# atoms-ufrj/atomsmm

Measured on AMD Instinct MI355X. Metric: ns/day on 100k-atom TIP3P RESPA box; near-nonbonded HBM GB/s vs 8 TB/s peak, higher is better.
Workload: dtype f64

## Files before the change

### atomsmm_amd/csrc/cluster.hip

```cpp
#include <algorithm>
#include <cmath>
#include <cstdio>
#include <cstdlib>
#include <cstring>
#include <type_traits>
#include <vector>

#include "amm_ctx.h"
#include "bonded_terms.h"
#include "cluster.h"
#include "device_utils.h"
#include "pair_math.h"
#include "pair_tab.h"

#ifndef AMM_EXP_NOLJ
#define AMM_EXP_NOLJ 0
#endif

__device__ double amm_erfcx_table_dev_c[AMM_ERFCX_NI * AMM_ERFCX_NC];
static bool g_erfcx_uploaded_c[64] = {false};

void amm_cluster_classify(int n, const std::vector<int> &ptr, const std::vector<int> &idx, std::vector<int> &mol_first, std::vector<int> &rest) {
    mol_first.clear();
    rest.clear();
// ... 813 lines not shown
                    const int T = __builtin_amdgcn_readfirstlane(s_cnt[0][t] + s_cnt[1][t] + s_cnt[2][t] + s_cnt[3][t]);
                    const int nch = (T + 127) >> 7;
                    const int have = __builtin_amdgcn_readlane(row_cnt, t);
                    int nf = have & 0xffff, nb_ = (int)((unsigned)have >> 16);
                    int *row_out = nl + (size_t)(tb + t - c_begin) * cap;
                    for (int k = 0; k < nch; ++k) {
                        const int j = j0 + k;
                        const int cc = __builtin_amdgcn_readfirstlane(s_ccnt[j]);
                        const int cn = cc & 0xffff, cf = (int)((unsigned)cc >> 16);
                        if ((j & 3) == w && nf + nb_ + cn + cf <= cap) {
                            for (int i = lane; i < cn; i += 64) row_out[nf + i] = s_stage[j][i];
                            for (int i = lane; i < cf; i += 64) row_out[cap - 1 - nb_ - i] = s_stage[j][127 - i];
                        }
                        nf = min(nf + cn, 0xffff);
                        nb_ = min(nb_ + cf, 0xffff);
                    }
                    row_cnt = lane == t ? (nf | (nb_ << 16)) : row_cnt;
                    j0 += nch;
                }
                CBS_STAMP(5);
                __syncthreads();
                CBS_STAMP(6);
            }
            if (w == 0 && lane < nt) {
                const int count = row_cnt & 0xffff, countf = (int)((unsigned)row_cnt >> 16);
                const int total_nb = count + countf;
                const bool over = total_nb > cap;
                nnb[tb + lane - c_begin] = over ? 0 : total_nb;
                nnb_near[tb + lane - c_begin] = over ? 0 : count;
                if (over) flags[1] = 1;
                wsum += (unsigned long long)total_nb;
                wnear += (unsigned long long)count;
                wmax = max(wmax, total_nb);
            }
        }
    }
    __syncthreads();
    }
    for (int off = 32; off > 0; off >>= 1) {
        wsum += __shfl_xor(wsum, off);
        wnear += __shfl_xor(wnear, off);
        wmax = max(wmax, __shfl_xor(wmax, off));
    }
    if (w == 0 && lane == 0) {
        amm_st_l2(&blockstats[3 * blockIdx.x], wsum);
        amm_st_l2(&blockstats[3 * blockIdx.x + 1], (unsigned long long)wmax);
        amm_st_l2(&blockstats[3 * blockIdx.x + 2], wnear);
    }
    if (amm_last_block(ticket)) cfinish_build_block(flags, counters, blockstats, (int)gridDim.x, 0);
}

#define AMM_CPHASES 6
struct CPairArgs {
    int c_begin, nrows, lpa_shift, cap;
    const int *aperm;
    const int *nl, *nnb, *nnb_total;
    const double4 *posq;
    const double2 *lj;
    double *force;
    int accumulate, sorted_out;
    Box box;
    const double *host_tab;
    int host_bytes;
    double margin;
    int ntask;
    int per_pair_image;
    int rpx, nphase;
    int ph_off[AMM_CPHASES], ph_shift[AMM_CPHASES], ph_ntask[AMM_CPHASES];
#ifdef AMM_CPAIR_TIMING
    unsigned long long *wave_times;
#endif
    const double *host_tab_ss;
    int host_ss_bytes, host_ss_off, site_atoms;
    double hsig_site, seps2_site;
    const double *guest_tab, *guest_tab_ss;
    int guest_bytes, guest_ss_bytes, guest_ss_off, g_accumulate;
    const double *tab_image;
    unsigned long long host_serial, guest_serial;
    PairForce *tab_owner;
    double *gforce;
    double gfac, gsr;
};

#ifdef AMM_CPAIR_TIMING
#define CWALK_T_PARAM , unsigned long long &t_first
#define CWALK_T_ARG , t_first
#else
#define CWALK_T_PARAM
#define CWALK_T_ARG
#endif
template <int FAM, int CMODE, int GFAM, int IMG, int SMASK>
__device__ __forceinline__ void cwalk_rows(const CPairArgs &A, const PairConsts &c, const PairConsts &g, const char *tabh, const char *tabg,
                                           const double *erfcx, const double4 (&pi)[3], const double2 *li, int i_sites, const int (&so)[3],
                                           const int (&sog)[3], double sign_lj, const int *row, int nfront, int nn, int sub, int lpa,
                                           int self, double (&f)[9], double (&fg)[9] CWALK_T_PARAM) {
    constexpr bool DUAL = GFAM >= 0;
    constexpr bool SS = SMASK != 0;
    const int back = A.cap - 1 + nfront;
    const double r2low = DUAL ? fmax(c.tab.r2min, g.tab.r2min) : c.tab.r2min;
    const double r2low_ss = DUAL ? fmax(c.tab.ss_r2min, g.tab.ss_r2min) : c.tab.ss_r2min;
    auto entry = [&](int k) { return k < nn ? row[k < nfront ? k : back - k] : self; };
    auto load_pos = [&](int e, int b) {
        return *reinterpret_cast<const double4 *>(reinterpret_cast<const char *>(A.posq) + (size_t)((unsigned)e & 0x1fffffffu) * 96u + 32 * b);
    };
    auto load_lj = [&](int e, int b) {
        double2 l = make_double2(0.0, 0.0);
        if (i_sites != 0 && __builtin_amdgcn_ballot_w64((((unsigned)e >> 29) >> b) & 1u) != 0ull)
            l = *reinterpret_cast<const double2 *>(reinterpret_cast<const char *>(A.lj) + (size_t)((unsigned)e & 0x1fffffffu) * 48u + 16 * b);
        return l;
    };
    double4 pj[3];
    double2 lj[3];
    int k = sub;
    int e = entry(k), en = entry(k + lpa);
#pragma unroll
    for (int b = 0; b < 3; ++b) {
        pj[b] = load_pos(e, b);
        if (!SS) lj[b] = load_lj(e, b);
    }
    while (__builtin_amdgcn_ballot_w64(k < nn) != 0ull) {
        const bool ok = k < nn;
        const bool front = k < nfront;
        const bool any_front = DUAL && __builtin_amdgcn_ballot_w64(front) != 0ull;
        const unsigned bits = (unsigned)e >> 29;
        const int e2 = entry(k + 2 * lpa);
        double sx = 0.0, sy = 0.0, sz = 0.0;
        if (IMG == 1) {
            sx = A.box.L[0] * rint((pj[0].x - pi[0].x) * A.box.invL[0]);
            sy = A.box.L[1] * rint((pj[0].y - pi[0].y) * A.box.invL[1]);
            sz = A.box.L[2] * rint((pj[0].z - pi[0].z) * A.box.invL[2]);
        }
#pragma unroll
        for (int b = 0; b < 3; ++b) {
            const double xb = pj[b].x - sx, yb = pj[b].y - sy, zb = pj[b].z - sz, qb = pj[b].w;
            const int mb = SS ? -(int)((bits >> b) & 1u) : 0;
            double dx[3], dy[3], dz[3], r2[3], fr[3], gl[3];
            {
                TabLookup th[3];
#pragma unroll
                for (int a = 0; a < 3; ++a) {
                    dx[a] = pi[a].x - xb;
                    dy[a] = pi[a].y - yb;
                    dz[a] = pi[a].z - zb;
                    if (IMG == 2) {
                        dx[a] = amm_min_image(dx[a], A.box.L[0], A.box.invL[0]);
                        dy[a] = amm_min_image(dy[a], A.box.L[1], A.box.invL[1]);
                        dz[a] = amm_min_image(dz[a], A.box.L[2], A.box.invL[2]);
                    }
                    r2[a] = dx[a] * dx[a] + dy[a] * dy[a] + dz[a] * dz[a];
                    th[a] = amm_tab_fetch(tabh, c.tab, r2[a], ((SMASK >> a) & 1) ? (unsigned)(so[a] & mb) : 0u);
                    if (DUAL) gl[a] = 0.0;
                }
                __builtin_amdgcn_sched_barrier(0);
#pragma unroll
                for (int a = 0; a < 3; ++a) fr[a] = (pi[a].w * qb) * amm_tab_horner(th[a]);
            }
            if (!SS && !AMM_EXP_NOLJ && i_sites != 0 && __builtin_amdgcn_ballot_w64(ok && ((bits >> b) & 1u)) != 0ull) {
#pragma unroll
                for (int a = 0; a < 3; ++a)
                    if ((i_sites >> a) & 1) {
                        const double2 la = li[64 * a];
                        const double sig = la.x + lj[b].x, eps4 = la.y * lj[b].y;
                        const LJCommon L = amm_lj_common(r2[a], sig, eps4);
                        fr[a] = amm_sum_unfused(fr[a], amm_lj_force<FAM, CMODE>(c, L, sig, eps4));
                        if (DUAL && any_front) {
                            LJCommon Lg = L;
                            Lg.dlj_r *= A.gsr;
                            gl[a] = amm_lj_force<(DUAL ? GFAM : FAM), 0>(g, Lg, sig, eps4 * A.gsr);
                        }
                    }
            }
            bool any_low = false;
            bool lowp[3];
#pragma unroll
            for (int a = 0; a < 3; ++a) {
                bool low = r2[a] < r2low;
                if ((SMASK >> a) & 1) low = low || ((so[a] & mb) != 0 && r2[a] < r2low_ss);
                lowp[a] = low;
                const bool pass = ok && (r2[a] < c.rc2);
                any_low = any_low || (ok && low);
                const double fh = (pass && !low) ? fr[a] : 0.0;
                f[3 * a] += fh * dx[a];
                f[3 * a + 1] += fh * dy[a];
                f[3 * a + 2] += fh * dz[a];
            }
            if (DUAL) {
                __builtin_amdgcn_sched_barrier(0);
                if (any_front) {
                    TabLookup tg[3];
#pragma unroll
                    for (int a = 0; a < 3; ++a) tg[a] = amm_tab_fetch(tabg, g.tab, r2[a], ((SMASK >> a) & 1) ? (unsigned)(sog[a] & mb) : 0u);
                    __builtin_amdgcn_sched_barrier(0);
#pragma unroll
                    for (int a = 0; a < 3; ++a) {
                        const double gr = amm_sum_unfused(((pi[a].w * qb) * A.gfac) * amm_tab_horner(tg[a]), gl[a]);
                        const bool pass = front && (r2[a] < g.rc2) && !lowp[a];
                        const double gh = pass ? gr : 0.0;
                        fg[3 * a] += gh * dx[a];
                        fg[3 * a + 1] += gh * dy[a];
                        fg[3 * a + 2] += gh * dz[a];
                    }
                }
            }
            if (__builtin_amdgcn_ballot_w64(any_low) != 0ull) {
                for (int a = 0; a < 3; ++a) {
                    const bool low = ok && lowp[a];
                    double sg, e4;
                    if (SS) {
                        const bool both = ((SMASK >> a) & 1) && (so[a] & mb) != 0;
                        sg = 2.0 * A.hsig_site;
                        e4 = both ? A.seps2_site * A.seps2_site * sign_lj : 0.0;
                    } else {
                        const double2 lx = A.lj[3 * ((unsigned)e & 0x1fffffffu) + b];
                        const double2 la = li[64 * a];
                        sg = la.x + lx.x;
                        e4 = la.y * lx.y;
                    }
                    double e_, fr_;
                    amm_pair_math<FAM, CMODE, false, false>(c, low ? r2[a] : 1.0, pi[a].w * qb, sg, e4, e_, fr_, erfcx);
                    fr_ = (low && r2[a] < c.rc2) ? fr_ : 0.0;
                    f[3 * a] += fr_ * dx[a];
                    f[3 * a + 1] += fr_ * dy[a];
                    f[3 * a + 2] += fr_ * dz[a];
                    if (DUAL) {
                        double gr_;
                        amm_pair_math<(DUAL ? GFAM : FAM), 0, false, false>(g, low ? r2[a] : 1.0, (pi[a].w * qb) * A.gfac, sg, e4 * A.gsr, e_, gr_, erfcx);
                        gr_ = (low && front && r2[a] < g.rc2) ? gr_ : 0.0;
                        fg[3 * a] += gr_ * dx[a];
                        fg[3 * a + 1] += gr_ * dy[a];
                        fg[3 * a + 2] += gr_ * dz[a];
                    }
                }
            }
            pj[b] = load_pos(en, b);
            if (!SS) lj[b] = load_lj(en, b);
        }
        e = en;
        en = e2;
        k += lpa;
#ifdef AMM_CPAIR_TIMING
        if (!t_first) t_first = wall_clock64();
#endif
    }
}

struct CEpiPre {
    const double *a, *b;
    double coef;
    int plus;
};
struct CEpiArgs {
    int niter, npre;
    int recompute_f0;
    double *x, *v, *f0;
    const double *mass;
    double c1, d, c2;
    CEpiPre pre[AMM_MAX_PRE];
    const int *cperm;
    const int4 *term_l;
    const double4 *term_q;
    const unsigned long long *atom_recs;
    int *spec_count, *spec_clear, *spec_members, *spec_start, *spec_flags, *spec_ticket;
    int spec_capc;
    CellGrid grid;
    double *xchg_x, *xchg_v;
    int c_first;
    double4 *posq_next;
    double2 *lj_next;
    const double *q_next, *hsig_next, *seps2_next;
    WatchArgs W;
};

#ifndef CEPI_INLINE
#define CEPI_INLINE __forceinline__
#endif

struct CEpiArgs;
template <int Q>
__device__ __forceinline__ double cquad_bcast(double v) {
    constexpr int ctrl = Q | (Q << 2) | (Q << 4) | (Q << 6);
    const long long b = __double_as_longlong(v);
    const int lo = __builtin_amdgcn_mov_dpp((int)(b & 0xffffffffll), ctrl, 0xf, 0xf, true);
    const int hi = __builtin_amdgcn_mov_dpp((int)(b >> 32), ctrl, 0xf, 0xf, true);
    return __longlong_as_double(((long long)hi << 32) | (unsigned int)lo);
}

struct PosTermRegs {
// ... 182 lines not shown
            AMM_CEPI_TERM(2)
            AMM_CEPI_TERM(3)
#undef AMM_CEPI_TERM
        }
        if (it >= 0) {
#pragma clang fp contract(off)
#pragma unroll
            for (int j = 0; j < 3; ++j) {
                const double num = E.c2 * f[j];
                const double dv = amm_div_mass(num, m, rm, rok);
                v[j] = v[j] + dv;
            }
        }
    }
    CEPI_STAMP(2);
    if (has) {
#pragma unroll
        for (int j = 0; j < 3; ++j) {
            if (E.niter == 0) E.x[3 * a + j] = x[j];
            E.v[3 * a + j] = v[j];
            E.f0[3 * a + j] = f[j];
        }
        if (E.xchg_x) {
            const size_t sl = 3 * (size_t)(cs - E.c_first) + l;
#pragma unroll
            for (int j = 0; j < 3; ++j) {
                if (E.niter == 0) E.xchg_x[3 * sl + j] = x[j];
                E.xchg_v[3 * sl + j] = v[j];
            }
        }
    }
}

template <int BS>
__device__ __forceinline__ int cscan_counts(int ncell, const int *count, int *start) {
    __shared__ int s_part[BS / 64], s_most[BS / 64];
    const int t = threadIdx.x, lane = t & 63, w = t >> 6;
    const int per = (ncell + BS - 1) / BS;
    const int c0 = min(t * per, ncell), c1 = min(c0 + per, ncell);
    int sum = 0, most = 0;
    for (int c = c0; c < c1; ++c) {
        const int v = amm_ld_l2(&count[c]);
        sum += v;
        most = max(most, v);
    }
    int incl = sum;
    for (int off = 1; off < 64; off <<= 1) {
        const int up = __shfl_up(incl, off);
        if (lane >= off) incl += up;
        most = max(most, __shfl_xor(most, off));
    }
    if (lane == 63) {
        s_part[w] = incl;
        s_most[w] = most;
    }
    __syncthreads();
    int base = 0, all_most = 0;
#pragma unroll
    for (int k = 0; k < BS / 64; ++k) {
        if (k < w) base += s_part[k];
        all_most = max(all_most, s_most[k]);
    }
    int run = base + incl - sum;
    for (int c = c0; c < c1; ++c) {
        start[c] = run;
        run += amm_ld_l2(&count[c]);
    }
    if (t == BS - 1) start[ncell] = run;
    return all_most;
}

#ifndef AMM_CBS_SINGLE
#define AMM_CBS_SINGLE 512
#endif

#ifndef AMM_CBS_NEAR
#define AMM_CBS_NEAR 512
#endif
#ifndef AMM_CTAB_WAVES_PER_EU
#define AMM_CTAB_WAVES_PER_EU 1
#endif
template <int FAM, int CMODE, int GFAM, int BS, int SMASK, bool EPI = false>
__global__ void __launch_bounds__(BS) __attribute__((amdgpu_waves_per_eu(AMM_CTAB_WAVES_PER_EU)))
k_cpair(CPairArgs A, PairConsts c, PairConsts g, CEpiArgs E) {
    constexpr bool DUAL = GFAM >= 0;
    constexpr bool SS = SMASK != 0;
    extern __shared__ __align__(16) char s_lds[];
    if (EPI && E.spec_clear) {
        for (int cidx = blockIdx.x * BS + threadIdx.x; cidx <= E.grid.ncell; cidx += gridDim.x * BS) E.spec_clear[cidx] = 0;
    }
#ifdef AMM_CPAIR_TIMING
    const unsigned long long t_entry = wall_clock64();
    unsigned long long t_staged = 0, t_first = 0;
    int n_tasks_done = 0, n_interior = 0;
    unsigned long long t_epi[3] = {0, 0, 0};
#endif
    constexpr int WPB = BS / 64;
    const int lane = threadIdx.x & 63;
    const double sign = c.sign;
    const int xcd = blockIdx.x & 7, nwx = (gridDim.x >> 3) * WPB;
    const int row_end = min((xcd + 1) * A.rpx, A.nrows);
#ifdef AMM_CPAIR_SWAP
    const int wave = (int)(threadIdx.x >> 6) ^ 4;
#else
    const int wave = (int)(threadIdx.x >> 6);
#endif
    const int task0 = (int)(blockIdx.x >> 3) * WPB + __builtin_amdgcn_readfirstlane(wave);
    int phase = 0, task = task0;
    auto seek = [&]() {
        while (phase < A.nphase && task >= A.ph_ntask[phase]) {
            ++phase;
            task = task0;
        }
        return phase < A.nphase;
    };
    constexpr bool AHEAD = SS;
    int shift = 0, lpa = 1, sub = 0, a = 0, cs = 0, nfront = 0, nn = 0;
    bool valid = false;
    const int *row = nullptr;
    double4 pi[3];
    double2 pl[3];
    auto pre_rows = [&]() {
        shift = A.ph_shift[phase];
        lpa = 1 << shift;
        sub = lane & (lpa - 1);
        a = xcd * A.rpx + A.ph_off[phase] + task * (64 >> shift) + (lane >> shift);
        valid = a < row_end;
        cs = A.c_begin + (valid ? a : 0);
#pragma unroll
        for (int t = 0; t < 3; ++t) {
            pi[t] = A.posq[3 * cs + t];
            pl[t] = A.lj[3 * cs + t];
        }
        nfront = valid ? A.nnb[a] : 0;
        nn = valid ? (A.nnb_total ? A.nnb_total[a] : nfront) : 0;
        row = A.nl + (size_t)(valid ? a : 0) * A.cap;
    };
    bool has = seek();
    if (AHEAD && has) pre_rows();

    const int used = A.host_bytes + (DUAL ? A.guest_bytes : 0) + (SS ? A.host_ss_bytes + (DUAL ? A.guest_ss_bytes : 0) : 0);
    double2 tabs[(160 * 1024) / (BS * 16)];
    amm_stage_issue<BS>(tabs, A.tab_image, used);
    amm_stage_commit<BS>(tabs, s_lds, used);
    amm_stage_rest<BS>(tabs, A.tab_image, s_lds, used);
#if defined(AMM_EXP_TAB_GLOBAL)
    const char *tabh = reinterpret_cast<const char *>(A.host_tab);
#else
    const char *tabh = s_lds;
#endif
    const char *tabg = s_lds + A.host_bytes;
    const double *erfcx = amm_erfcx_table_dev_c;
    double2 *s_li = nullptr;
    if (!SS) {
        double *s_erfcx = reinterpret_cast<double *>(s_lds + used);
        for (int k = threadIdx.x; k < AMM_ERFCX_NI * AMM_ERFCX_NC; k += BS) s_erfcx[k] = amm_erfcx_table_dev_c[k];
        erfcx = s_erfcx;
        s_li = reinterpret_cast<double2 *>(s_erfcx + AMM_ERFCX_NI * AMM_ERFCX_NC) + (threadIdx.x >> 6) * 192;
    }
    __syncthreads();
#ifdef AMM_CPAIR_TIMING
    t_staged = wall_clock64();
#endif

    PairConsts c1 = c, g1 = g;
    c1.sign = 1.0;
    g1.sign = 1.0;
    while (has) {
        if (!AHEAD) pre_rows();
        const int t_a = a, t_cs = cs, t_sub = sub, t_lpa = lpa;
        const bool t_valid = valid;
        int i_sites = 0;
        int so[3] = {0, 0, 0}, sog[3] = {0, 0, 0};
        if (!SS) __builtin_amdgcn_wave_barrier();
#pragma unroll
        for (int t = 0; t < 3; ++t) {
            pi[t].w *= c.Kc * sign;
            double2 l = pl[t];
            l.y *= sign;
            if (!SS) s_li[64 * t + lane] = l;
            const bool site = valid && l.y != 0.0;
            if ((SMASK >> t) & 1) {
                so[t] = site ? A.host_ss_off : 0;
                if (DUAL) sog[t] = site ? A.guest_ss_off : 0;
            }
            if (__builtin_amdgcn_ballot_w64(site) != 0ull) i_sites |= 1 << t;
        }
        if (!SS) {
            __builtin_amdgcn_fence(__ATOMIC_RELEASE, "wavefront");
            __builtin_amdgcn_wave_barrier();
            __builtin_amdgcn_fence(__ATOMIC_ACQUIRE, "wavefront");
        }
        const double2 *li = SS ? nullptr : s_li + lane;
        const bool edge = valid && !(pi[0].x >= A.margin && pi[0].x <= A.box.L[0] - A.margin && pi[0].y >= A.margin &&
                                     pi[0].y <= A.box.L[1] - A.margin && pi[0].z >= A.margin && pi[0].z <= A.box.L[2] - A.margin);
        const bool interior = __builtin_amdgcn_ballot_w64(edge) == 0ull;
#ifdef AMM_CPAIR_TIMING
        ++n_tasks_done;
        n_interior += interior ? 1 : 0;
#endif
        double f[9], fg[9];
#pragma unroll
        for (int k = 0; k < 9; ++k) f[k] = fg[k] = 0.0;
        if (A.per_pair_image) cwalk_rows<FAM, CMODE, GFAM, 2, SMASK>(A, c1, g1, tabh, tabg, erfcx, pi, li, i_sites, so, sog, sign, row, nfront, nn, sub, lpa, cs, f, fg CWALK_T_ARG);
        else if (interior) cwalk_rows<FAM, CMODE, GFAM, 0, SMASK>(A, c1, g1, tabh, tabg, erfcx, pi, li, i_sites, so, sog, sign, row, nfront, nn, sub, lpa, cs, f, fg CWALK_T_ARG);
        else cwalk_rows<FAM, CMODE, GFAM, 1, SMASK>(A, c1, g1, tabh, tabg, erfcx, pi, li, i_sites, so, sog, sign, row, nfront, nn, sub, lpa, cs, f, fg CWALK_T_ARG);
        task += nwx;
        has = seek();
        if (AHEAD && has) pre_rows();
        for (int off = t_lpa >> 1; off > 0; off >>= 1) {
#pragma unroll
            for (int k = 0; k < 9; ++k) {
                f[k] += __shfl_xor(f[k], off);
                if (DUAL) fg[k] += __shfl_xor(fg[k], off);
            }
        }
        if (t_valid && t_sub == 0) {
#pragma unroll
            for (int t = 0; t < 3; ++t) {
                const int i = A.sorted_out ? 3 * t_a + t : A.aperm[3 * t_cs + t];
#pragma unroll
                for (int d = 0; d < 3; ++d) {
                    if (A.accumulate) A.force[3 * i + d] += f[3 * t + d];
                    else A.force[3 * i + d] = f[3 * t + d];
                    if (DUAL) {
                        if (A.g_accumulate) A.gforce[3 * i + d] += fg[3 * t + d];
                        else A.gforce[3 * i + d] = fg[3 * t + d];
                    }
                }
            }
        }
    }
#ifdef AMM_CPAIR_TIMING
    if (EPI) t_staged = wall_clock64();
#endif
    if (EPI) {
        for (int phase = 0; phase < A.nphase; ++phase) {
            const int shift = A.ph_shift[phase], row0 = xcd * A.rpx + A.ph_off[phase], ntask = A.ph_ntask[phase];
            const int rpw = 64 >> shift;
            for (int task = (int)(blockIdx.x >> 3) * WPB + (int)(threadIdx.x >> 6); task < ntask; task += nwx) {
                const int a = row0 + task * rpw + (lane >> shift);
                const bool valid = a < row_end;
#ifdef AMM_CPAIR_TIMING
                cepi_rows(E, A.box, A.c_begin + (valid ? a : 0), valid, lane & ((1 << shift) - 1), t_epi);
#else
                cepi_rows(E, A.box, A.c_begin + (valid ? a : 0), valid, lane & ((1 << shift) - 1));
#endif
            }
        }
        if (E.spec_count && amm_last_block(E.spec_ticket)) {
            if (amm_ld_l2(&E.spec_flags[0])) {
                const int fullest = cscan_counts<BS>(E.grid.ncell, E.spec_count, E.spec_start);
                if (threadIdx.x == 0) E.spec_flags[6] = fullest;
            }
        }
    }
#ifdef AMM_CPAIR_TIMING
    if (A.wave_times && (threadIdx.x & 63) == 0) {
        unsigned long long *o = A.wave_times + 4 * ((size_t)blockIdx.x * (BS / 64) + (threadIdx.x >> 6));
        o[0] = t_entry;
        o[1] = t_staged;
        o[2] = wall_clock64();
        o[3] = EPI ? (((t_epi[0] - t_staged) & 0xfffffull) | (((t_epi[1] - t_staged) & 0xfffffull) << 20) | (((t_epi[2] - t_staged) & 0xfffffull) << 40))
                   : ((((t_first ? t_first - t_entry : 0ull) & 0xfffffull) << 24) | ((unsigned long long)(n_interior & 0xffff) << 8) | (unsigned long long)(n_tasks_done & 0xff));
    }
#endif
}

static const double AMM_PHASE_COST[7] = {0, 0, 1.0, 0.55, 0.32, 0.18, 0.11};
static double cpair_plan_rec(int rows, int waves, int s, int off, CPairArgs *P) {
    const int rpw = 64 >> s, per_round = waves * rpw;
    const int full = rows / per_round, left = rows - full * per_round;
    const double finish = (double)((rows + per_round - 1) / per_round) * AMM_PHASE_COST[s];
    auto put = [&](int ntask) {
        if (P && ntask > 0) {
            P->ph_off[P->nphase] = off;
            P->ph_shift[P->nphase] = s;
            P->ph_ntask[P->nphase] = ntask;
            ++P->nphase;
        }
    };
    int s2 = 6;
    double split = 1e300;
    for (int t = s + 1; t <= 6 && left > 0; ++t) {
        const double v = cpair_plan_rec(left, waves, t, 0, nullptr);
        if (v < split) {
            split = v;
            s2 = t;
        }
    }
    split += full * AMM_PHASE_COST[s];
    if (left == 0 || s == 6 || finish <= split) {
        put((rows + rpw - 1) / rpw);
        return finish;
    }
    put(full * waves);
    cpair_plan_rec(left, waves, s2, off + full * per_round, P);
    return split;
}
static void cpair_plan(CPairArgs &P, int waves, int enabled) {
    P.rpx = (P.nrows + 7) / 8;
    P.nphase = 0;
    if (enabled) {
        cpair_plan_rec(P.rpx, waves, P.lpa_shift, 0, &P);
    } else {
        const int rpw = 64 >> P.lpa_shift;
        P.ph_off[0] = 0;
        P.ph_shift[0] = P.lpa_shift;
        P.ph_ntask[0] = (P.rpx + rpw - 1) / rpw;
        P.nphase = 1;
    }
}

static int cpair_tab_image(amm_ctx *ctx, CPairArgs &P, bool dual, bool ss) {
    const void *src[4] = {P.host_tab, dual ? P.guest_tab : nullptr, ss ? P.host_tab_ss : nullptr, (ss && dual) ? P.guest_tab_ss : nullptr};
    const int len[4] = {P.host_bytes, dual ? P.guest_bytes : 0, ss ? P.host_ss_bytes : 0, (ss && dual) ? P.guest_ss_bytes : 0};
    const unsigned long long gs = dual ? P.guest_serial : 0;
    const size_t bytes = (size_t)len[0] + len[1] + len[2] + len[3];
    PairForce::TabImage &im = P.tab_owner->tab_image[(dual ? 1 : 0) | (ss ? 2 : 0)];
    if (!(im.d && im.host_serial == P.host_serial && im.guest_serial == gs && im.bytes == bytes && im.stream == ctx->stream)) {
        im.host_serial = 0;
        if (im.d && im.stream != ctx->stream) AMM_HIP(hipDeviceSynchronize());
        if (im.bytes != bytes) {
            if (im.d) (void)hipFree(im.d);
            im.d = nullptr;
            im.bytes = 0;
            AMM_HIP(hipMalloc(&im.d, bytes));
            im.bytes = bytes;
        }
        size_t at = 0;
        for (int k = 0; k < 4; ++k) {
            if (len[k] > 0) AMM_HIP(hipMemcpyAsync(im.d + at, src[k], (size_t)len[k], hipMemcpyDeviceToDevice, ctx->stream));
            at += (size_t)len[k];
        }
        im.stream = ctx->stream;
        im.guest_serial = gs;
        im.host_serial = P.host_serial;
    }
    P.tab_image = reinterpret_cast<const double *>(im.d);
    return 0;
}

// ... 854 lines not shown
```

### atomsmm_amd/csrc/pair.hip

```cpp
#include <atomic>
#include <cmath>
#include <cstdio>
#include <cstdlib>
#include <cstring>

#include "amm_ctx.h"
#include "bonded_terms.h"
#include "cluster.h"
#include "device_utils.h"
#include "pair_args.h"
#include "pair_math.h"
#include "pair_tab.h"

int amm_pair_build_consts(const amm_pair_desc &d, PairConsts &pc) {
    pc.family = d.family;
    pc.flags = d.flags;
    pc.degree = d.degree < 1 ? 1 : d.degree;
    pc.cmode = (d.flags & AMM_COULOMB_EWALD) ? 1 : ((d.flags & AMM_COULOMB_RF) ? 2 : 0);
    pc.sign = d.sign;
    pc.rc = d.rc;
    pc.rc2 = d.rc * d.rc;
    pc.rc0 = d.rc0;
    pc.rs0 = d.rs0;
    pc.inv_dr0 = (d.rc0 > d.rs0) ? 1.0 / (d.rc0 - d.rs0) : 0.0;
// ... 1880 lines not shown
}

bool amm_pair_can_eval_dual(amm_ctx *ctx, PairForce *guest, PairForce *host) {
    if (!guest || !host || guest->host != host || host->host) return false;
    if (guest->dual_ok >= 0) return guest->dual_ok == 1;
    guest->dual_ok = 0;
    const int gf = guest->desc.family, hf = host->desc.family;
    if (!(gf == AMM_NEAR_NONE || gf == AMM_NEAR_SHIFT || gf == AMM_NEAR_FSWITCH)) return false;
    if (!(hf == AMM_DAMPED || hf == AMM_NONBONDED)) return false;
    if ((guest->desc.flags & AMM_GUARD_RC0) || (host->desc.flags & AMM_GUARD_RC0)) return false;
    if ((guest->desc.flags | host->desc.flags) & (AMM_GROUP_LJ | AMM_GROUP_Q)) return false;
    if (!(guest->desc.rc <= host->desc.rc)) return false;
    if (guest->pc.Kc != host->pc.Kc) return false;
    const size_t n = (size_t)ctx->n;
    std::vector<double> a(n), b(n);
    const double *ga[3] = {guest->d_q, guest->d_hsig, guest->d_seps2}, *ha[3] = {host->d_q, host->d_hsig, host->d_seps2};
    for (int k = 0; k < 3; ++k) {
        if (hipMemcpy(a.data(), ga[k], sizeof(double) * n, hipMemcpyDeviceToHost) != hipSuccess) return false;
        if (hipMemcpy(b.data(), ha[k], sizeof(double) * n, hipMemcpyDeviceToHost) != hipSuccess) return false;
        if (std::memcmp(a.data(), b.data(), sizeof(double) * n) != 0) return false;
    }
    guest->dual_ok = 1;
    return true;
}

__global__ void __launch_bounds__(256) k_count_within(PairArgs A, double r2w, int nslice, unsigned long long *out) {
    const int tid = blockIdx.x * blockDim.x + threadIdx.x;
    const int a = tid >> A.lpa_shift, sub = tid & ((1 << A.lpa_shift) - 1);
    unsigned long long cnt = 0;
    if (a < nslice) {
        const int s = A.s_begin + a;
        const double4 pi = A.posq_s[s];
        const int nfront = A.nnb[a], nn = A.nnb_total ? A.nnb_total[a] : nfront;
        const int *row = A.nl + (size_t)a * A.cap;
        const int back = A.cap - 1 + nfront;
        for (int k = sub; k < nn; k += 1 << A.lpa_shift) {
            const double4 pj = A.posq_s[row[k < nfront ? k : back - k]];
            const double dx = amm_min_image(pi.x - pj.x, A.box.L[0], A.box.invL[0]);
            const double dy = amm_min_image(pi.y - pj.y, A.box.L[1], A.box.invL[1]);
            const double dz = amm_min_image(pi.z - pj.z, A.box.L[2], A.box.invL[2]);
            cnt += (dx * dx + dy * dy + dz * dz < r2w) ? 1ull : 0ull;
        }
    }
    for (int off = 32; off > 0; off >>= 1) cnt += __shfl_xor(cnt, off);
    if ((threadIdx.x & 63) == 0 && cnt) atomicAdd(out, cnt);
}

int amm_pair_count_within_impl(amm_ctx *ctx, PairForce *pf, const double *d_pos, double r_within, long long *count) {
    PairForce *L = pf->host ? pf->host : pf;
    if (!L->built) {
        amm_set_error("amm_pair_count_within: evaluate the force once first (the neighbour rows do not exist yet)");
        return 1;
    }
    hipStream_t st = ctx->stream;
    const int n = pf->n;
    hipLaunchKernelGGL(k_gather_sorted, dim3((n + 255) / 256), dim3(256), 0, st, n, L->d_perm, d_pos, pf->d_q, pf->d_hsig,
                       pf->d_seps2, ctx->box, pf->d_posq_s, pf->d_lj_s);
    PairArgs A;
    std::memset(&A, 0, sizeof(A));
    A.s_begin = L->s_begin;
    A.s_end = L->s_end;
    A.lpa_shift = 3;
    A.cap = L->cap;
    A.nl = L->d_nl;
    A.nnb = L->d_nnb_near;
    A.nnb_total = (pf == L && L->rnear_build > 0) ? L->d_nnb : nullptr;
    A.posq_s = pf->d_posq_s;
    A.box = ctx->box;
    const int nslice = L->s_end - L->s_begin;
    unsigned long long *d_cnt = L->d_counters + 7;
    AMM_HIP(hipMemsetAsync(d_cnt, 0, sizeof(unsigned long long), st));
    if (nslice > 0)
        hipLaunchKernelGGL(k_count_within, dim3((unsigned)(((long)nslice * 8 + 255) / 256)), dim3(256), 0, st, A, r_within * r_within, nslice, d_cnt);
    unsigned long long h = 0;
    AMM_HIP(hipMemcpyAsync(&h, d_cnt, sizeof(h), hipMemcpyDeviceToHost, st));
    AMM_HIP(hipStreamSynchronize(st));
    *count = (long long)h;
    return 0;
}

extern "C" __attribute__((weak)) const char *amm_variant_tag(void);
const char *amm_kernel_revision_impl() {
#ifdef AMM_CLUSTER_TUNE
    return "r06-prologue-tune";
#else
    return amm_variant_tag ? "r06-prologue-tune" : "r06-prologue";
#endif
}

int amm_pair_build_table(PairForce *pf) {
    std::vector<double> coef;
    SiteTable ss;
    ss.want = pf->cluster_ok && pf->one_site_class && pf->site_one_charge && pf->site_q != 0.0 && pf->site_seps2 != 0.0;
    ss.sig = 2.0 * pf->site_hsig;
    ss.eps4 = pf->site_seps2 * pf->site_seps2;
    ss.QQ = pf->pc.Kc * pf->site_q * pf->site_q;
    pf->tab_error = amm_build_coulomb_table(pf->pc, coef, &ss);
    pf->ss_built_for[0] = pf->site_hsig;
    pf->ss_built_for[1] = pf->site_seps2;
    pf->ss_built_for[2] = ss.want ? pf->site_q : 0.0;
    if (pf->d_tab) {
        (void)hipFree(pf->d_tab);
        pf->d_tab = nullptr;
    }
    if (pf->d_tab_ss) {
        (void)hipFree(pf->d_tab_ss);
        pf->d_tab_ss = nullptr;
    }
    pf->ss_error = ss.error;
    static std::atomic<unsigned long long> uploads{0};
    pf->tab_serial = ++uploads;
    if (pf->pc.tab.nint > 0 && !(pf->tab_error <= AMM_TAB_MAX_ERROR)) {
        pf->pc.tab.nint = 0;
        coef.clear();
    }
    if (pf->pc.tab.nint == 0 || ss.coef.empty() || !(ss.error <= AMM_TAB_SS_MAX_ERROR)) {
        pf->pc.tab.ss_first = -1;
        ss.coef.clear();
    }
    if (pf->pc.tab.nint > 0) {
        AMM_HIP(hipMalloc(&pf->d_tab, sizeof(double) * coef.size()));
        AMM_HIP(hipMemcpy(pf->d_tab, coef.data(), sizeof(double) * coef.size(), hipMemcpyHostToDevice));
    }
    if (!ss.coef.empty()) {
        AMM_HIP(hipMalloc(&pf->d_tab_ss, sizeof(double) * ss.coef.size()));
        AMM_HIP(hipMemcpy(pf->d_tab_ss, ss.coef.data(), sizeof(double) * ss.coef.size(), hipMemcpyHostToDevice));
    }
    return 0;
}

bool amm_pair_can_fuse_discount(amm_ctx *ctx, PairForce *guest, PairForce *host) {
    if (!guest || !host || guest->host != host || host->host) return false;
    if (!(guest->desc.flags & AMM_GUARD_RC0)) return false;
    if (guest->fuse_ok >= 0) return guest->fuse_ok == 1;
    guest->fuse_ok = 0;
    if (!ctx->opt_tab) return false;
    const int gf = guest->desc.family, hf = host->desc.family;
    if (!(gf == AMM_NEAR_NONE || gf == AMM_NEAR_SHIFT || gf == AMM_NEAR_FSWITCH)) return false;
    if (!(hf == AMM_DAMPED || hf == AMM_NONBONDED)) return false;
    if ((host->desc.flags & AMM_GUARD_RC0) || host->pc.sign != 1.0) return false;
    if ((guest->desc.flags | host->desc.flags) & (AMM_GROUP_LJ | AMM_GROUP_Q)) return false;
    if (!(guest->pc.tab.nint > 0 && guest->d_tab && host->pc.tab.nint > 0 && host->d_tab)) return false;
    if (guest->pc.Kc != host->pc.Kc) return false;
    const size_t n = (size_t)ctx->n;
    std::vector<double> a(n), b(n);
    const double *ga[3] = {guest->d_q, guest->d_hsig, guest->d_seps2}, *ha[3] = {host->d_q, host->d_hsig, host->d_seps2};
    for (int k = 0; k < 3; ++k) {
        if (hipMemcpy(a.data(), ga[k], sizeof(double) * n, hipMemcpyDeviceToHost) != hipSuccess) return false;
        if (hipMemcpy(b.data(), ha[k], sizeof(double) * n, hipMemcpyDeviceToHost) != hipSuccess) return false;
        if (std::memcmp(a.data(), b.data(), sizeof(double) * n) != 0) return false;
    }
    guest->fuse_ok = 1;
    return true;
}

int amm_pair_free(PairForce *pf) {
    void *ptrs[] = {pf->d_q, pf->d_hsig, pf->d_seps2, pf->d_excl_ptr, pf->d_excl_idx, pf->d_cell_of, pf->d_cell_count,
                    pf->d_cell_start, pf->d_cell_members, pf->d_perm, pf->d_posq_s, pf->d_lj_s, pf->d_xref,
                    pf->d_nl, pf->d_nnb, pf->d_flags, pf->d_counters, pf->d_epart, pf->d_pos4f_s, pf->d_blockstats, pf->d_inv_perm, pf->d_nnb_near, pf->d_nl_out, pf->d_nnb_out,
                    pf->d_nnb_scratch, pf->d_xref_out, pf->d_ticket, pf->d_tab, pf->d_cls, pf->d_cell_count_lj, pf->d_cell_start_lj,
                    pf->d_row_order, pf->d_member, pf->d_active, pf->d_cell_sets, pf->d_nnb_lj, pf->d_mol_first, pf->d_rest_idx};
    for (void *p : ptrs)
        if (p) (void)hipFree(p);
    for (PairForce::TabImage &im : pf->tab_image) {
        if (im.d) (void)hipFree(im.d);
        im = PairForce::TabImage();
    }
    for (hipEvent_t e : pf->ev) (void)hipEventDestroy(e);
    if (pf->cl) amm_cluster_free(pf->cl);
// ... 39 lines not shown
```

Measured before the change: 1098.

## Reload kernel args from kernarg segment and pin hot values in VGPRs

Kernel arguments are no longer kept live across the main loop. They are re-read from the kernarg segment through an opaque pointer where needed, including inside the rare low-r branch. Selected table constants, lpa and the posq pointer are forced into VGPRs for most template instantiations, which frees SGPRs and shortens live ranges in the triple-site pair loop. The low-r detection uses wave ballots instead of a per-lane OR in the non-dual case, and the SS path skips adding an unused LJ term. This trades extra scalar loads for lower register pressure, and the inline-asm register pinning could also hurt scheduling.

```diff
diff --git a/atomsmm_amd/csrc/cluster.hip b/atomsmm_amd/csrc/cluster.hip
--- a/atomsmm_amd/csrc/cluster.hip
+++ b/atomsmm_amd/csrc/cluster.hip
@@ -919,6 +919,36 @@
     double gfac, gsr;
 };
 
+struct CPairKArgs {
+    CPairArgs A;
+    PairConsts c, g;
+};
+static_assert(alignof(CPairArgs) == 8 && alignof(PairConsts) == 8 && sizeof(CPairArgs) % 8 == 0 && sizeof(PairConsts) % 8 == 0,
+              "CPairKArgs must lay out k_cpair's arguments as the kernarg segment does");
+typedef const __attribute__((address_space(4))) CPairKArgs *CPairKArgsP;
+__device__ __forceinline__ CPairKArgsP cpair_args_here() {
+    int zero = 0;
+    asm volatile("" : "+s"(zero));
+    return (CPairKArgsP)((const __attribute__((address_space(4))) char *)__builtin_amdgcn_kernarg_segment_ptr() + zero);
+}
+template <bool ON = true, class T>
+__device__ __forceinline__ T cpair_in_vgpr(T x) {
+    if (ON) asm("" : "+v"(x));
+    return x;
+}
+#ifndef AMM_TRIP_VGPR
+#define AMM_TRIP_VGPR 1
+#endif
+constexpr bool cpair_vgpr_room(int fam, int cmode, int gfam, int smask) {
+    return AMM_TRIP_VGPR != 0 && !(fam == AMM_DAMPED && cmode == 0) && !(fam == AMM_NONBONDED && cmode == 1 && gfam >= 0 && smask != 1);
+}
+template <class T>
+__device__ __forceinline__ T cpair_arg_copy(const __attribute__((address_space(4))) T *src) {
+    T out;
+    __builtin_memcpy(&out, src, sizeof(T));
+    return out;
+}
+
 #ifdef AMM_CPAIR_TIMING
 #define CWALK_T_PARAM , unsigned long long &t_first
 #define CWALK_T_ARG , t_first
@@ -929,16 +959,22 @@
 template <int FAM, int CMODE, int GFAM, int IMG, int SMASK>
 __device__ __forceinline__ void cwalk_rows(const CPairArgs &A, const PairConsts &c, const PairConsts &g, const char *tabh, const char *tabg,
                                            const double *erfcx, const double4 (&pi)[3], const double2 *li, int i_sites, const int (&so)[3],
-                                           const int (&sog)[3], double sign_lj, const int *row, int nfront, int nn, int sub, int lpa,
+                                           const int (&sog)[3], const int *row, int nfront, int nn, int sub, int lpa_s,
                                            int self, double (&f)[9], double (&fg)[9] CWALK_T_PARAM) {
     constexpr bool DUAL = GFAM >= 0;
     constexpr bool SS = SMASK != 0;
+    typedef double cwalk_d4 __attribute__((ext_vector_type(4)));
+    typedef const __attribute__((address_space(1))) char *cwalk_gptr;
+    constexpr bool VRES = cpair_vgpr_room(FAM, CMODE, GFAM, SMASK);
+    const int lpa = cpair_in_vgpr<VRES>(lpa_s);
+    const cwalk_gptr posq = (cwalk_gptr)cpair_in_vgpr<VRES>((unsigned long long)A.posq);
     const int back = A.cap - 1 + nfront;
     const double r2low = DUAL ? fmax(c.tab.r2min, g.tab.r2min) : c.tab.r2min;
     const double r2low_ss = DUAL ? fmax(c.tab.ss_r2min, g.tab.ss_r2min) : c.tab.ss_r2min;
     auto entry = [&](int k) { return k < nn ? row[k < nfront ? k : back - k] : self; };
     auto load_pos = [&](int e, int b) {
-        return *reinterpret_cast<const double4 *>(reinterpret_cast<const char *>(A.posq) + (size_t)((unsigned)e & 0x1fffffffu) * 96u + 32 * b);
+        const cwalk_d4 p = *(const __attribute__((address_space(1))) cwalk_d4 *)(posq + (size_t)((unsigned)e & 0x1fffffffu) * 96u + 32 * b);
+        return make_double4(p.x, p.y, p.z, p.w);
     };
     auto load_lj = [&](int e, int b) {
         double2 l = make_double2(0.0, 0.0);
@@ -957,6 +993,7 @@
     }
     while (__builtin_amdgcn_ballot_w64(k < nn) != 0ull) {
         const bool ok = k < nn;
+        const unsigned long long okm = __builtin_amdgcn_ballot_w64(ok);
         const bool front = k < nfront;
         const bool any_front = DUAL && __builtin_amdgcn_ballot_w64(front) != 0ull;
         const unsigned bits = (unsigned)e >> 29;
@@ -1007,16 +1044,24 @@
                         }
                     }
             }
+            constexpr bool LOW_MASKS = !DUAL;
+            unsigned long long lowm = 0ull;
             bool any_low = false;
             bool lowp[3];
 #pragma unroll
             for (int a = 0; a < 3; ++a) {
-                bool low = r2[a] < r2low;
-                if ((SMASK >> a) & 1) low = low || ((so[a] & mb) != 0 && r2[a] < r2low_ss);
+                const bool low_c = r2[a] < r2low;
+                bool low = low_c;
+                if (LOW_MASKS) lowm |= __builtin_amdgcn_ballot_w64(low_c);
+                if ((SMASK >> a) & 1) {
+                    const bool site_pair = (so[a] & mb) != 0, low_ss = r2[a] < r2low_ss;
+                    low = low | (site_pair & low_ss);
+                    if (LOW_MASKS) lowm |= __builtin_amdgcn_ballot_w64(site_pair) & __builtin_amdgcn_ballot_w64(low_ss);
+                }
                 lowp[a] = low;
-                const bool pass = ok && (r2[a] < c.rc2);
-                any_low = any_low || (ok && low);
-                const double fh = (pass && !low) ? fr[a] : 0.0;
+                const bool pass = ok & (r2[a] < c.rc2) & !low;
+                if (!LOW_MASKS) any_low = any_low | (ok & low);
+                const double fh = pass ? fr[a] : 0.0;
                 f[3 * a] += fh * dx[a];
                 f[3 * a + 1] += fh * dy[a];
                 f[3 * a + 2] += fh * dz[a];
@@ -1030,8 +1075,9 @@
                     __builtin_amdgcn_sched_barrier(0);
 #pragma unroll
                     for (int a = 0; a < 3; ++a) {
-                        const double gr = amm_sum_unfused(((pi[a].w * qb) * A.gfac) * amm_tab_horner(tg[a]), gl[a]);
-                        const bool pass = front && (r2[a] < g.rc2) && !lowp[a];
+                        double gr = ((pi[a].w * qb) * A.gfac) * amm_tab_horner(tg[a]);
+                        if (!SS) gr = amm_sum_unfused(gr, gl[a]);
+                        const bool pass = front & (r2[a] < g.rc2) & !lowp[a];
                         const double gh = pass ? gr : 0.0;
                         fg[3 * a] += gh * dx[a];
                         fg[3 * a + 1] += gh * dy[a];
@@ -1039,7 +1085,12 @@
                     }
                 }
             }
-            if (__builtin_amdgcn_ballot_w64(any_low) != 0ull) {
+            if (LOW_MASKS ? (lowm & okm) != 0ull : __builtin_amdgcn_ballot_w64(any_low) != 0ull) {
+                const CPairKArgsP K = cpair_args_here();
+                const CPairArgs A = cpair_arg_copy(&K->A);
+                PairConsts c = cpair_arg_copy(&K->c), g = cpair_arg_copy(&K->g);
+                const double sign_lj = c.sign;
+                c.sign = g.sign = 1.0;
                 for (int a = 0; a < 3; ++a) {
                     const bool low = ok && lowp[a];
                     double sg, e4;
@@ -1388,7 +1439,7 @@
 #endif
 template <int FAM, int CMODE, int GFAM, int BS, int SMASK, bool EPI = false>
 __global__ void __launch_bounds__(BS) __attribute__((amdgpu_waves_per_eu(AMM_CTAB_WAVES_PER_EU)))
-k_cpair(CPairArgs A, PairConsts c, PairConsts g, CEpiArgs E) {
+k_cpair(CPairArgs A_, PairConsts c_, PairConsts g_, CEpiArgs E) {
     constexpr bool DUAL = GFAM >= 0;
     constexpr bool SS = SMASK != 0;
     extern __shared__ __align__(16) char s_lds[];
@@ -1403,9 +1454,13 @@
 #endif
     constexpr int WPB = BS / 64;
     const int lane = threadIdx.x & 63;
-    const double sign = c.sign;
     const int xcd = blockIdx.x & 7, nwx = (gridDim.x >> 3) * WPB;
-    const int row_end = min((xcd + 1) * A.rpx, A.nrows);
+    int row_end, rpx;
+    {
+        const CPairKArgsP K = cpair_args_here();
+        rpx = K->A.rpx;
+        row_end = min((xcd + 1) * rpx, K->A.nrows);
+    }
 #ifdef AMM_CPAIR_SWAP
     const int wave = (int)(threadIdx.x >> 6) ^ 4;
 #else
@@ -1414,11 +1469,13 @@
     const int task0 = (int)(blockIdx.x >> 3) * WPB + __builtin_amdgcn_readfirstlane(wave);
     int phase = 0, task = task0;
     auto seek = [&]() {
-        while (phase < A.nphase && task >= A.ph_ntask[phase]) {
+        const CPairKArgsP K = cpair_args_here();
+        const int nphase = K->A.nphase;
+        while (phase < nphase && task >= K->A.ph_ntask[phase]) {
             ++phase;
             task = task0;
         }
-        return phase < A.nphase;
+        return phase < nphase;
     };
     constexpr bool AHEAD = SS;
     int shift = 0, lpa = 1, sub = 0, a = 0, cs = 0, nfront = 0, nn = 0;
@@ -1427,35 +1484,46 @@
     double4 pi[3];
     double2 pl[3];
     auto pre_rows = [&]() {
-        shift = A.ph_shift[phase];
+        const CPairKArgsP K = cpair_args_here();
+        const double4 *posq = K->A.posq;
+        const double2 *ljp = K->A.lj;
+        const int *nnb = K->A.nnb, *nnb_total = K->A.nnb_total;
+        shift = K->A.ph_shift[phase];
         lpa = 1 << shift;
         sub = lane & (lpa - 1);
-        a = xcd * A.rpx + A.ph_off[phase] + task * (64 >> shift) + (lane >> shift);
+        a = xcd * rpx + K->A.ph_off[phase] + task * (64 >> shift) + (lane >> shift);
         valid = a < row_end;
-        cs = A.c_begin + (valid ? a : 0);
+        cs = K->A.c_begin + (valid ? a : 0);
 #pragma unroll
         for (int t = 0; t < 3; ++t) {
-            pi[t] = A.posq[3 * cs + t];
-            pl[t] = A.lj[3 * cs + t];
-        }
-        nfront = valid ? A.nnb[a] : 0;
-        nn = valid ? (A.nnb_total ? A.nnb_total[a] : nfront) : 0;
-        row = A.nl + (size_t)(valid ? a : 0) * A.cap;
+            pi[t] = posq[3 * cs + t];
+            pl[t] = ljp[3 * cs + t];
+        }
+        nfront = valid ? nnb[a] : 0;
+        nn = valid ? (nnb_total ? nnb_total[a] : nfront) : 0;
+        row = K->A.nl + (size_t)(valid ? a : 0) * K->A.cap;
     };
     bool has = seek();
     if (AHEAD && has) pre_rows();
 
-    const int used = A.host_bytes + (DUAL ? A.guest_bytes : 0) + (SS ? A.host_ss_bytes + (DUAL ? A.guest_ss_bytes : 0) : 0);
-    double2 tabs[(160 * 1024) / (BS * 16)];
-    amm_stage_issue<BS>(tabs, A.tab_image, used);
-    amm_stage_commit<BS>(tabs, s_lds, used);
-    amm_stage_rest<BS>(tabs, A.tab_image, s_lds, used);
+    const char *tabh, *tabg;
+    int used;
+    {
+        const CPairKArgsP K = cpair_args_here();
+        const int host_bytes = K->A.host_bytes;
+        used = host_bytes + (DUAL ? K->A.guest_bytes : 0) + (SS ? K->A.host_ss_bytes + (DUAL ? K->A.guest_ss_bytes : 0) : 0);
+        const double *tab_image = K->A.tab_image;
+        double2 tabs[(160 * 1024) / (BS * 16)];
+        amm_stage_issue<BS>(tabs, tab_image, used);
+        amm_stage_commit<BS>(tabs, s_lds, used);
+        amm_stage_rest<BS>(tabs, tab_image, s_lds, used);
 #if defined(AMM_EXP_TAB_GLOBAL)
-    const char *tabh = reinterpret_cast<const char *>(A.host_tab);
+        tabh = reinterpret_cast<const char *>(K->A.host_tab);
 #else
-    const char *tabh = s_lds;
-#endif
-    const char *tabg = s_lds + A.host_bytes;
+        tabh = s_lds;
+#endif
+        tabg = s_lds + host_bytes;
+    }
     const double *erfcx = amm_erfcx_table_dev_c;
     double2 *s_li = nullptr;
     if (!SS) {
@@ -1469,11 +1537,25 @@
     t_staged = wall_clock64();
 #endif
 
-    PairConsts c1 = c, g1 = g;
-    c1.sign = 1.0;
-    g1.sign = 1.0;
     while (has) {
         if (!AHEAD) pre_rows();
+        const CPairKArgsP K = cpair_args_here();
+        const CPairArgs A = cpair_arg_copy(&K->A);
+        PairConsts c1 = cpair_arg_copy(&K->c), g1 = cpair_arg_copy(&K->g);
+        const double sign = c1.sign, Kc = c1.Kc;
+        c1.sign = 1.0;
+        g1.sign = 1.0;
+        constexpr bool VRES = cpair_vgpr_room(FAM, CMODE, GFAM, SMASK);
+        c1.tab.shiftB = cpair_in_vgpr<VRES>(c1.tab.shiftB);
+        c1.tab.rawB_minus_nA = cpair_in_vgpr<VRES>(c1.tab.rawB_minus_nA);
+        c1.tab.baseA = cpair_in_vgpr<VRES>(c1.tab.baseA);
+        c1.tab.halfB = cpair_in_vgpr<VRES>(c1.tab.halfB);
+        if (DUAL) {
+            g1.tab.shiftB = cpair_in_vgpr<VRES>(g1.tab.shiftB);
+            g1.tab.rawB_minus_nA = cpair_in_vgpr<VRES>(g1.tab.rawB_minus_nA);
+            g1.tab.baseA = cpair_in_vgpr<VRES>(g1.tab.baseA);
+            g1.tab.halfB = cpair_in_vgpr<VRES>(g1.tab.halfB);
+        }
         const int t_a = a, t_cs = cs, t_sub = sub, t_lpa = lpa;
         const bool t_valid = valid;
         int i_sites = 0;
@@ -1481,7 +1563,7 @@
         if (!SS) __builtin_amdgcn_wave_barrier();
 #pragma unroll
         for (int t = 0; t < 3; ++t) {
-            pi[t].w *= c.Kc * sign;
+            pi[t].w *= Kc * sign;
             double2 l = pl[t];
             l.y *= sign;
             if (!SS) s_li[64 * t + lane] = l;
@@ -1508,9 +1590,9 @@
         double f[9], fg[9];
 #pragma unroll
         for (int k = 0; k < 9; ++k) f[k] = fg[k] = 0.0;
-        if (A.per_pair_image) cwalk_rows<FAM, CMODE, GFAM, 2, SMASK>(A, c1, g1, tabh, tabg, erfcx, pi, li, i_sites, so, sog, sign, row, nfront, nn, sub, lpa, cs, f, fg CWALK_T_ARG);
-        else if (interior) cwalk_rows<FAM, CMODE, GFAM, 0, SMASK>(A, c1, g1, tabh, tabg, erfcx, pi, li, i_sites, so, sog, sign, row, nfront, nn, sub, lpa, cs, f, fg CWALK_T_ARG);
-        else cwalk_rows<FAM, CMODE, GFAM, 1, SMASK>(A, c1, g1, tabh, tabg, erfcx, pi, li, i_sites, so, sog, sign, row, nfront, nn, sub, lpa, cs, f, fg CWALK_T_ARG);
+        if (A.per_pair_image) cwalk_rows<FAM, CMODE, GFAM, 2, SMASK>(A, c1, g1, tabh, tabg, erfcx, pi, li, i_sites, so, sog, row, nfront, nn, sub, lpa, cs, f, fg CWALK_T_ARG);
+        else if (interior) cwalk_rows<FAM, CMODE, GFAM, 0, SMASK>(A, c1, g1, tabh, tabg, erfcx, pi, li, i_sites, so, sog, row, nfront, nn, sub, lpa, cs, f, fg CWALK_T_ARG);
+        else cwalk_rows<FAM, CMODE, GFAM, 1, SMASK>(A, c1, g1, tabh, tabg, erfcx, pi, li, i_sites, so, sog, row, nfront, nn, sub, lpa, cs, f, fg CWALK_T_ARG);
         task += nwx;
         has = seek();
         if (AHEAD && has) pre_rows();
@@ -1522,16 +1604,20 @@
             }
         }
         if (t_valid && t_sub == 0) {
+            const CPairKArgsP Ks = cpair_args_here();
+            const int sorted_out = Ks->A.sorted_out, accumulate = Ks->A.accumulate, g_accumulate = Ks->A.g_accumulate;
+            const int *aperm = Ks->A.aperm;
+            double *force = Ks->A.force, *gforce = Ks->A.gforce;
 #pragma unroll
             for (int t = 0; t < 3; ++t) {
-                const int i = A.sorted_out ? 3 * t_a + t : A.aperm[3 * t_cs + t];
+                const int i = sorted_out ? 3 * t_a + t : aperm[3 * t_cs + t];
 #pragma unroll
                 for (int d = 0; d < 3; ++d) {
-                    if (A.accumulate) A.force[3 * i + d] += f[3 * t + d];
-                    else A.force[3 * i + d] = f[3 * t + d];
+                    if (accumulate) force[3 * i + d] += f[3 * t + d];
+                    else force[3 * i + d] = f[3 * t + d];
                     if (DUAL) {
-                        if (A.g_accumulate) A.gforce[3 * i + d] += fg[3 * t + d];
-                        else A.gforce[3 * i + d] = fg[3 * t + d];
+                        if (g_accumulate) gforce[3 * i + d] += fg[3 * t + d];
+                        else gforce[3 * i + d] = fg[3 * t + d];
                     }
                 }
             }
@@ -1541,16 +1627,19 @@
     if (EPI) t_staged = wall_clock64();
 #endif
     if (EPI) {
-        for (int phase = 0; phase < A.nphase; ++phase) {
-            const int shift = A.ph_shift[phase], row0 = xcd * A.rpx + A.ph_off[phase], ntask = A.ph_ntask[phase];
+        const CPairKArgsP K = cpair_args_here();
+        const int nphase = K->A.nphase, c_begin = K->A.c_begin;
+        const Box box = cpair_arg_copy(&K->A.box);
+        for (int phase = 0; phase < nphase; ++phase) {
+            const int shift = K->A.ph_shift[phase], row0 = xcd * rpx + K->A.ph_off[phase], ntask = K->A.ph_ntask[phase];
             const int rpw = 64 >> shift;
             for (int task = (int)(blockIdx.x >> 3) * WPB + (int)(threadIdx.x >> 6); task < ntask; task += nwx) {
                 const int a = row0 + task * rpw + (lane >> shift);
                 const bool valid = a < row_end;
 #ifdef AMM_CPAIR_TIMING
-                cepi_rows(E, A.box, A.c_begin + (valid ? a : 0), valid, lane & ((1 << shift) - 1), t_epi);
+                cepi_rows(E, box, c_begin + (valid ? a : 0), valid, lane & ((1 << shift) - 1), t_epi);
 #else
-                cepi_rows(E, A.box, A.c_begin + (valid ? a : 0), valid, lane & ((1 << shift) - 1));
+                cepi_rows(E, box, c_begin + (valid ? a : 0), valid, lane & ((1 << shift) - 1));
 #endif
             }
         }
@@ -1562,8 +1651,8 @@
         }
     }
 #ifdef AMM_CPAIR_TIMING
-    if (A.wave_times && (threadIdx.x & 63) == 0) {
-        unsigned long long *o = A.wave_times + 4 * ((size_t)blockIdx.x * (BS / 64) + (threadIdx.x >> 6));
+    if (A_.wave_times && (threadIdx.x & 63) == 0) {
+        unsigned long long *o = A_.wave_times + 4 * ((size_t)blockIdx.x * (BS / 64) + (threadIdx.x >> 6));
         o[0] = t_entry;
         o[1] = t_staged;
         o[2] = wall_clock64();
diff --git a/atomsmm_amd/csrc/pair.hip b/atomsmm_amd/csrc/pair.hip
--- a/atomsmm_amd/csrc/pair.hip
+++ b/atomsmm_amd/csrc/pair.hip
@@ -1986,9 +1986,9 @@
 extern "C" __attribute__((weak)) const char *amm_variant_tag(void);
 const char *amm_kernel_revision_impl() {
 #ifdef AMM_CLUSTER_TUNE
-    return "r06-prologue-tune";
+    return "r07-triploop-tune";
 #else
-    return amm_variant_tag ? "r06-prologue-tune" : "r06-prologue";
+    return amm_variant_tag ? "r07-triploop-tune" : "r07-triploop";
 #endif
 }
 
```

After: 1156 (median of 6 runs). +5.3%, better.
